# chiy48308/audio_feature_extraction

Measured on AMD Instinct MI355X. Metric: audio frames/sec (sr=22050, n_fft=1024, hop=256, n_mfcc=13), higher is better.
Workload: dtype f32; 1 GPU; 1000x10s clips @22050 Hz per GPU, frame_length=1024, hop_length=256, n_mfcc=13, n_mels=128, hamming, pre-emphasis 0.97 + trim 30 dB + RMS (BASELINE configs[1]); clips_per_gpu=1000, frames_per_gpu_step=862000, input=HBM-resident float32

## Files before the change

### audio_feature_extraction_amd/csrc/afx_trim3.hip

```cpp
#include <hip/hip_runtime.h>

#include "afx_device.h"
#include "afx_frames3.h"
#include "afx_trim_dev.h"
#include "afx_wave.h"

namespace afx {

__global__ __launch_bounds__(256) void k_trim_decide3(const ClipDesc* __restrict__ clips, ClipInfo* __restrict__ info,
                                                      const float* __restrict__ bsum, const float* __restrict__ blockmax,
                                                      BlockDesc* __restrict__ items, int* __restrict__ n_items, int max_items,
                                                      float* __restrict__ rms_rows, KParams kp) {
  __shared__ float red_f[4];
  __shared__ long long red_a[4], red_b[4];
  const int clip = blockIdx.x, tid = threadIdx.x, wave = tid >> 6, lane = tid & 63;
  const ClipDesc cd = clips[clip];
  const int64_t N = cd.len;
  const uint32_t nonfinite = info[clip].nonfinite;
  int status = AFX_CLIP_OK;
  if (N < 2) status = AFX_CLIP_TOO_SHORT;
  else if (nonfinite) status = AFX_CLIP_NONFINITE;
  int64_t start = 0, end = N;
  const int per = kp.rms_sub;
  if ((kp.flags & AFX_FLAG_TRIM) && status == AFX_CLIP_OK)
    trim_search(bsum + cd.tblk_base * per, N, kp, per, red_f, red_a, red_b, true, start, end);
  const int hop = kp.hop;
  const int T = (int)(1 + (end - start) / hop);
  if (status == AFX_CLIP_OK && T < 9) status = AFX_CLIP_TOO_SHORT;
  const int g0 = (int)(start / hop), glast = g0 + T - 1;
  const int nblk = cd.tpad / kFramesPerBlock;
  const bool cutL = start > 0, cutR = end < N;
  const int bLo = cutL ? (g0 + 2 + 15) >> 4 : 0;
  const int bHi = cutR ? (glast >= 17 ? (glast - 17) >> 4 : -1) : nblk - 1;
  float cm = -INFINITY;
  if (status == AFX_CLIP_OK)
    for (int b = bLo + tid; b <= bHi; b += 256) cm = fmaxf(cm, blockmax[cd.blk_base + b]);
  cm = wave_max(cm);
  if (lane == 0) red_f[wave] = cm;
  __syncthreads();
  cm = fmaxf(fmaxf(red_f[0], red_f[1]), fmaxf(red_f[2], red_f[3]));
  if (tid == 0) {
    ClipInfo ci;
    ci.start = start; ci.end = end; ci.T = T; ci.status = status;
    ci.lmax_ord = cm > -INFINITY ? f2ord(cm) : 0u;
    ci.nonfinite = nonfinite;
    info[clip] = ci;
    if (status == AFX_CLIP_OK && (cutL || cutR)) {
      int r0[2], r1[2], nr = 0;
      if (bLo > bHi) { r0[0] = g0; r1[0] = glast + 1; nr = 1; }
      else {
        if (cutL && 16 * bLo > g0) { r0[nr] = g0; r1[nr] = 16 * bLo < glast + 1 ? 16 * bLo : glast + 1; ++nr; }
        if (cutR && 16 * (bHi + 1) <= glast) { r0[nr] = 16 * (bHi + 1) > g0 ? 16 * (bHi + 1) : g0; r1[nr] = glast + 1; ++nr; }
      }
      int cnt = 0;
      for (int r = 0; r < nr; ++r) cnt += (r1[r] - r0[r] + 15) / 16;
      if (cnt > 0) {
        const int at = atomicAdd(n_items, cnt);
        int k = 0;
        for (int r = 0; r < nr; ++r)
          for (int gf = r0[r]; gf < r1[r]; gf += 16, ++k) {
            if (at + k >= max_items) break;
            const int nfr = r1[r] - gf < 16 ? r1[r] - gf : 16;
            items[at + k] = make_block(cd, clip, (int64_t)gf * hop - kp.n_fft / 2, gf, start, end, N, 0, nfr, true, 0, 0);
          }
      }
    }
  }
  if (rms_rows && (status == AFX_CLIP_OK || (status == AFX_CLIP_TOO_SHORT && N >= 2)))
    trim_rms_rows(bsum + cd.tblk_base * per, start, end, T, kp, rms_rows + cd.frame_base);
}

__global__ __launch_bounds__(64) void k_build_blocks3(const ClipDesc* __restrict__ clips, int n_clips,
                                                      BlockDesc* __restrict__ blocks, int n_fft, int hop, int trim_hop, int per) {
  const int clip = blockIdx.x;
  if (clip >= n_clips) return;
  const ClipDesc c = clips[clip];
  const int nb = c.tpad / kFramesPerBlock;
  const int64_t ntb = (c.len + trim_hop - 1) / trim_hop;
  for (int b = threadIdx.x; b < nb; b += 64) {
    const int64_t gs = (int64_t)b * kFramesPerBlock * hop - n_fft / 2;
    const int t0 = b * kFramesPerBlock;
    blocks[c.blk_base + b] = make_block(c, clip, gs, t0, 0, c.len, c.len, t0, c.tmax, c.len >= 2 && t0 < c.tmax,
                                        (int32_t)(c.tblk_base * per), (int32_t)(ntb * per));
  }
}

hipError_t launch_build_blocks3(hipStream_t s, const ClipDesc* clips, int n_clips, int nblocks, BlockDesc* blocks,
                                const KParams& kp) {
  if (nblocks <= 0 || n_clips <= 0) return hipSuccess;
  hipLaunchKernelGGL(k_build_blocks3, dim3(n_clips), dim3(64), 0, s, clips, n_clips, blocks,
                     kp.n_fft, kp.hop, kp.trim_hop, kp.rms_sub);
  return hipGetLastError();
}

hipError_t launch_trim_decide3(hipStream_t s, const ClipDesc* clips, ClipInfo* info, const float* bsum, const float* blockmax,
                               BlockDesc* items, int* n_items, int max_items, float* rms_rows, int n_clips, const KParams& kp) {
  hipLaunchKernelGGL(k_trim_decide3, dim3(n_clips), dim3(256), 0, s, clips, info, bsum, blockmax, items, n_items, max_items,
                     rms_rows, kp);
  return hipGetLastError();
}

}
```

### audio_feature_extraction_amd/csrc/afx_trim_dev.h

```cpp
#pragma once
#include "afx_device.h"
#include "afx_wave.h"

namespace afx {

__device__ __forceinline__ float trim_frame_rms(const float* bs, int64_t t, int64_t nb, int half, int per, float inv_n) {
  float s = 0.f;
  for (int64_t b = (t - half) * per; b < (t + half) * per; ++b)
    if (b >= 0 && b < nb * per) s += bs[b];
  return sqrtf(s * inv_n);
}

__device__ __forceinline__ void trim_search(const float* bs, int64_t N, const KParams& kp, int per, float* red_f,
                                            long long* red_a, long long* red_b, bool reuse_red_f, int64_t& start, int64_t& end) {
  const int tid = threadIdx.x, wave = tid >> 6, lane = tid & 63;
  const int th = kp.trim_hop, half = (kp.trim_frame / th) / 2;
  const int64_t nb = (N + th - 1) / th, nt = 1 + N / th;
  const float inv_n = 1.0f / (float)kp.trim_frame;
  float mx = 0.f;
  for (int64_t t = tid; t < nt; t += 256) mx = fmaxf(mx, trim_frame_rms(bs, t, nb, half, per, inv_n));
  mx = wave_max(mx);
  if (lane == 0) red_f[wave] = mx;
  __syncthreads();
  mx = fmaxf(fmaxf(red_f[0], red_f[1]), fmaxf(red_f[2], red_f[3]));
  if (reuse_red_f) __syncthreads();
  const float ref_db = 10.0f * log10f(fmaxf(1e-10f, mx * mx));
  long long first = (long long)1 << 62, last = -1;
  for (int64_t t = tid; t < nt; t += 256) {
    const float r = trim_frame_rms(bs, t, nb, half, per, inv_n);
    const float db = 10.0f * log10f(fmaxf(1e-10f, r * r)) - ref_db;
    if (db > -kp.trim_top_db) { if (t < first) first = t; if (t > last) last = t; }
  }
#pragma unroll
  for (int o = 32; o >= 1; o >>= 1) {
    const long long f2 = __shfl_xor(first, o), l2 = __shfl_xor(last, o);
    first = f2 < first ? f2 : first; last = l2 > last ? l2 : last;
  }
  if (lane == 0) { red_a[wave] = first; red_b[wave] = last; }
  __syncthreads();
  first = red_a[0]; last = red_b[0];
#pragma unroll
  for (int w = 1; w < 4; ++w) { first = red_a[w] < first ? red_a[w] : first; last = red_b[w] > last ? red_b[w] : last; }
  if (last >= 0) {
    start = first * th;
    end = (last + 1) * th < N ? (last + 1) * th : N;
  } else { start = 0; end = 0; }
}

__device__ __forceinline__ void trim_rms_rows(const float* bs, int64_t start, int64_t end, int T, const KParams& kp, float* rows) {
  const int64_t s_lo = start / kp.hop, s_hi = (end + kp.hop - 1) / kp.hop;
  const int nsb = kp.n_fft / kp.hop, back = nsb / 2;
  const float inv_n = 1.0f / (float)kp.n_fft;
  for (int t = threadIdx.x; t < T; t += 256) {
    float sacc = 0.f;
    for (int k = 0; k < nsb; ++k) {
      const int64_t sb = s_lo + t - back + k;
      if (sb >= s_lo && sb < s_hi) sacc += bs[sb];
    }
    rows[t] = sqrtf(sacc * inv_n);
  }
}

}
```

Baseline: 1.420 billion frames/s.

## Process one clip per wavefront in trim-decide kernel and batch window-sum loads

The trim-decide kernel now gives each 64-lane wavefront its own clip, four clips per 256-thread block, in place of a whole block per clip. This removes the shared-memory reductions and __syncthreads. The blockmax read is prefetched per lane, and the window sums for trim RMS and frame RMS now issue 8 predicated loads at a time so more memory requests are in flight. In exchange, each clip gets a quarter as many threads for its trim scan and RMS rows, which lengthens per-clip latency.

```diff
diff --git a/audio_feature_extraction_amd/csrc/afx_trim3.hip b/audio_feature_extraction_amd/csrc/afx_trim3.hip
--- a/audio_feature_extraction_amd/csrc/afx_trim3.hip
+++ b/audio_feature_extraction_amd/csrc/afx_trim3.hip
@@ -7,39 +7,40 @@
 
 namespace afx {
 
-__global__ __launch_bounds__(256) void k_trim_decide3(const ClipDesc* __restrict__ clips, ClipInfo* __restrict__ info,
+constexpr int kDecideWaves = 4;
+
+__global__ __launch_bounds__(kDecideWaves * 64) void k_trim_decide3(const ClipDesc* __restrict__ clips, ClipInfo* __restrict__ info,
                                                       const float* __restrict__ bsum, const float* __restrict__ blockmax,
                                                       BlockDesc* __restrict__ items, int* __restrict__ n_items, int max_items,
-                                                      float* __restrict__ rms_rows, KParams kp) {
-  __shared__ float red_f[4];
-  __shared__ long long red_a[4], red_b[4];
-  const int clip = blockIdx.x, tid = threadIdx.x, wave = tid >> 6, lane = tid & 63;
+                                                      float* __restrict__ rms_rows, KParams kp, int n_clips) {
+  const int wave = threadIdx.x >> 6, lane = threadIdx.x & 63;
+  const int clip = blockIdx.x * kDecideWaves + wave;
+  if (clip >= n_clips) return;
   const ClipDesc cd = clips[clip];
   const int64_t N = cd.len;
+  const int per = kp.rms_sub, hop = kp.hop;
+  const int nblk = cd.tpad / kFramesPerBlock;
+  const float* const bs = bsum + cd.tblk_base * per;
   const uint32_t nonfinite = info[clip].nonfinite;
+  const float bm_lane = lane < nblk ? blockmax[cd.blk_base + lane] : -INFINITY;
   int status = AFX_CLIP_OK;
   if (N < 2) status = AFX_CLIP_TOO_SHORT;
   else if (nonfinite) status = AFX_CLIP_NONFINITE;
   int64_t start = 0, end = N;
-  const int per = kp.rms_sub;
   if ((kp.flags & AFX_FLAG_TRIM) && status == AFX_CLIP_OK)
-    trim_search(bsum + cd.tblk_base * per, N, kp, per, red_f, red_a, red_b, true, start, end);
-  const int hop = kp.hop;
+    trim_search_wave(bs, N, kp, per, start, end);
   const int T = (int)(1 + (end - start) / hop);
   if (status == AFX_CLIP_OK && T < 9) status = AFX_CLIP_TOO_SHORT;
   const int g0 = (int)(start / hop), glast = g0 + T - 1;
-  const int nblk = cd.tpad / kFramesPerBlock;
   const bool cutL = start > 0, cutR = end < N;
   const int bLo = cutL ? (g0 + 2 + 15) >> 4 : 0;
   const int bHi = cutR ? (glast >= 17 ? (glast - 17) >> 4 : -1) : nblk - 1;
   float cm = -INFINITY;
   if (status == AFX_CLIP_OK)
-    for (int b = bLo + tid; b <= bHi; b += 256) cm = fmaxf(cm, blockmax[cd.blk_base + b]);
+    for (int b = lane; b < nblk; b += 64)
+      if (b >= bLo && b <= bHi) cm = fmaxf(cm, b == lane ? bm_lane : blockmax[cd.blk_base + b]);
   cm = wave_max(cm);
-  if (lane == 0) red_f[wave] = cm;
-  __syncthreads();
-  cm = fmaxf(fmaxf(red_f[0], red_f[1]), fmaxf(red_f[2], red_f[3]));
-  if (tid == 0) {
+  if (lane == 0) {
     ClipInfo ci;
     ci.start = start; ci.end = end; ci.T = T; ci.status = status;
     ci.lmax_ord = cm > -INFINITY ? f2ord(cm) : 0u;
@@ -67,7 +68,7 @@
     }
   }
   if (rms_rows && (status == AFX_CLIP_OK || (status == AFX_CLIP_TOO_SHORT && N >= 2)))
-    trim_rms_rows(bsum + cd.tblk_base * per, start, end, T, kp, rms_rows + cd.frame_base);
+    trim_rms_rows(bs, start, end, T, kp, rms_rows + cd.frame_base, lane, 64);
 }
 
 __global__ __launch_bounds__(64) void k_build_blocks3(const ClipDesc* __restrict__ clips, int n_clips,
@@ -95,8 +96,9 @@
 
 hipError_t launch_trim_decide3(hipStream_t s, const ClipDesc* clips, ClipInfo* info, const float* bsum, const float* blockmax,
                                BlockDesc* items, int* n_items, int max_items, float* rms_rows, int n_clips, const KParams& kp) {
-  hipLaunchKernelGGL(k_trim_decide3, dim3(n_clips), dim3(256), 0, s, clips, info, bsum, blockmax, items, n_items, max_items,
-                     rms_rows, kp);
+  if (n_clips <= 0) return hipSuccess;
+  hipLaunchKernelGGL(k_trim_decide3, dim3((n_clips + kDecideWaves - 1) / kDecideWaves), dim3(kDecideWaves * 64), 0, s, clips, info, bsum,
+                     blockmax, items, n_items, max_items, rms_rows, kp, n_clips);
   return hipGetLastError();
 }
 
diff --git a/audio_feature_extraction_amd/csrc/afx_trim_dev.h b/audio_feature_extraction_amd/csrc/afx_trim_dev.h
--- a/audio_feature_extraction_amd/csrc/afx_trim_dev.h
+++ b/audio_feature_extraction_amd/csrc/afx_trim_dev.h
@@ -4,59 +4,96 @@
 
 namespace afx {
 
+__device__ __forceinline__ float window_sum(const float* bs, int64_t b0, int n, int64_t lo, int64_t hi) {
+  float s = 0.f;
+  for (int k0 = 0; k0 < n; k0 += 8) {
+    float v[8];
+#pragma unroll
+    for (int j = 0; j < 8; ++j) {
+      const int64_t b = b0 + k0 + j;
+      const bool in = k0 + j < n && b >= lo && b < hi;
+      v[j] = bs[in ? b : 0];
+      v[j] = in ? v[j] : 0.f;
+    }
+#pragma unroll
+    for (int j = 0; j < 8; ++j) s += v[j];
+  }
+  return s;
+}
+
 __device__ __forceinline__ float trim_frame_rms(const float* bs, int64_t t, int64_t nb, int half, int per, float inv_n) {
-  float s = 0.f;
-  for (int64_t b = (t - half) * per; b < (t + half) * per; ++b)
-    if (b >= 0 && b < nb * per) s += bs[b];
-  return sqrtf(s * inv_n);
+  return sqrtf(window_sum(bs, (t - half) * per, 2 * half * per, 0, nb * per) * inv_n);
 }
+
+struct TrimWalk {
+  int th, half, per;
+  int64_t nb, nt;
+  float inv_n;
+  __device__ TrimWalk(int64_t N, const KParams& kp, int per_)
+      : th(kp.trim_hop), half((kp.trim_frame / kp.trim_hop) / 2), per(per_), nb((N + kp.trim_hop - 1) / kp.trim_hop),
+        nt(1 + N / kp.trim_hop), inv_n(1.0f / (float)kp.trim_frame) {}
+  __device__ __forceinline__ float peak(const float* bs, int tid, int nth) const {
+    float mx = 0.f;
+    for (int64_t t = tid; t < nt; t += nth) mx = fmaxf(mx, trim_frame_rms(bs, t, nb, half, per, inv_n));
+    return mx;
+  }
+  __device__ __forceinline__ void span(const float* bs, float mx, float top_db, int tid, int nth, long long& first, long long& last) const {
+    const float ref_db = 10.0f * log10f(fmaxf(1e-10f, mx * mx));
+    first = (long long)1 << 62; last = -1;
+    for (int64_t t = tid; t < nt; t += nth) {
+      const float r = trim_frame_rms(bs, t, nb, half, per, inv_n);
+      const float db = 10.0f * log10f(fmaxf(1e-10f, r * r)) - ref_db;
+      if (db > -top_db) { if (t < first) first = t; if (t > last) last = t; }
+    }
+#pragma unroll
+    for (int o = 32; o >= 1; o >>= 1) {
+      const long long f2 = __shfl_xor(first, o), l2 = __shfl_xor(last, o);
+      first = f2 < first ? f2 : first; last = l2 > last ? l2 : last;
+    }
+  }
+  __device__ __forceinline__ void cut(long long first, long long last, int64_t N, int64_t& start, int64_t& end) const {
+    if (last >= 0) {
+      start = first * th;
+      end = (last + 1) * th < N ? (last + 1) * th : N;
+    } else { start = 0; end = 0; }
+  }
+};
 
 __device__ __forceinline__ void trim_search(const float* bs, int64_t N, const KParams& kp, int per, float* red_f,
                                             long long* red_a, long long* red_b, bool reuse_red_f, int64_t& start, int64_t& end) {
   const int tid = threadIdx.x, wave = tid >> 6, lane = tid & 63;
-  const int th = kp.trim_hop, half = (kp.trim_frame / th) / 2;
-  const int64_t nb = (N + th - 1) / th, nt = 1 + N / th;
-  const float inv_n = 1.0f / (float)kp.trim_frame;
-  float mx = 0.f;
-  for (int64_t t = tid; t < nt; t += 256) mx = fmaxf(mx, trim_frame_rms(bs, t, nb, half, per, inv_n));
-  mx = wave_max(mx);
+  const TrimWalk w(N, kp, per);
+  float mx = wave_max(w.peak(bs, tid, 256));
   if (lane == 0) red_f[wave] = mx;
   __syncthreads();
   mx = fmaxf(fmaxf(red_f[0], red_f[1]), fmaxf(red_f[2], red_f[3]));
   if (reuse_red_f) __syncthreads();
-  const float ref_db = 10.0f * log10f(fmaxf(1e-10f, mx * mx));
-  long long first = (long long)1 << 62, last = -1;
-  for (int64_t t = tid; t < nt; t += 256) {
-    const float r = trim_frame_rms(bs, t, nb, half, per, inv_n);
-    const float db = 10.0f * log10f(fmaxf(1e-10f, r * r)) - ref_db;
-    if (db > -kp.trim_top_db) { if (t < first) first = t; if (t > last) last = t; }
-  }
-#pragma unroll
-  for (int o = 32; o >= 1; o >>= 1) {
-    const long long f2 = __shfl_xor(first, o), l2 = __shfl_xor(last, o);
-    first = f2 < first ? f2 : first; last = l2 > last ? l2 : last;
-  }
+  long long first, last;
+  w.span(bs, mx, kp.trim_top_db, tid, 256, first, last);
   if (lane == 0) { red_a[wave] = first; red_b[wave] = last; }
   __syncthreads();
   first = red_a[0]; last = red_b[0];
 #pragma unroll
-  for (int w = 1; w < 4; ++w) { first = red_a[w] < first ? red_a[w] : first; last = red_b[w] > last ? red_b[w] : last; }
-  if (last >= 0) {
-    start = first * th;
-    end = (last + 1) * th < N ? (last + 1) * th : N;
-  } else { start = 0; end = 0; }
+  for (int i = 1; i < 4; ++i) { first = red_a[i] < first ? red_a[i] : first; last = red_b[i] > last ? red_b[i] : last; }
+  w.cut(first, last, N, start, end);
 }
 
-__device__ __forceinline__ void trim_rms_rows(const float* bs, int64_t start, int64_t end, int T, const KParams& kp, float* rows) {
+__device__ __forceinline__ void trim_search_wave(const float* bs, int64_t N, const KParams& kp, int per, int64_t& start, int64_t& end) {
+  const int lane = threadIdx.x & 63;
+  const TrimWalk w(N, kp, per);
+  const float mx = wave_max(w.peak(bs, lane, 64));
+  long long first, last;
+  w.span(bs, mx, kp.trim_top_db, lane, 64, first, last);
+  w.cut(first, last, N, start, end);
+}
+
+__device__ __forceinline__ void trim_rms_rows(const float* bs, int64_t start, int64_t end, int T, const KParams& kp, float* rows,
+                                              int tid = threadIdx.x, int nth = 256) {
   const int64_t s_lo = start / kp.hop, s_hi = (end + kp.hop - 1) / kp.hop;
   const int nsb = kp.n_fft / kp.hop, back = nsb / 2;
   const float inv_n = 1.0f / (float)kp.n_fft;
-  for (int t = threadIdx.x; t < T; t += 256) {
-    float sacc = 0.f;
-    for (int k = 0; k < nsb; ++k) {
-      const int64_t sb = s_lo + t - back + k;
-      if (sb >= s_lo && sb < s_hi) sacc += bs[sb];
-    }
+  for (int t = tid; t < T; t += nth) {
+    const float sacc = window_sum(bs, s_lo + t - back, nsb, s_lo, s_hi);
     rows[t] = sqrtf(sacc * inv_n);
   }
 }
```

Result: no change. 1.422 billion frames/s, median of 6 (+0.1%).
